# b51/ceres_mono_orb_slam2

Measured on AMD Instinct MI355X. Metric: frames/sec ORB extract+match @1241x376 + LocalBA solves/sec; 1/2/4/8 GPU, higher is better.
Workload: dtype u8; 1 GPU; KITTI 1241x376, 2000 features/frame requested (nfeatures = 2000), 8 levels, ORB extract + brute-force Hamming match vs previous frame (ratio 0.9, TH_LOW 50, rotation histogram); frames_per_launch=256, streams=2

## Files before the change

ceres_mono_orb_slam2_amd/csrc/orb_extractor.hip:

```cpp
#include <hip/hip_runtime.h>
#include <cmath>
#include <cstdint>
#include <cstdlib>
#include <atomic>
#include <vector>
#include <algorithm>
#include <new>
#include <type_traits>

#include "common.h"
#include "orb_pattern_data.h"

namespace orbhip {

static const int PATCH_SIZE = 31, HALF_PATCH = 15, EDGE_THRESHOLD = 19;
static const int MAX_LEVELS = 16;
static const int MAX_INI = 64;
static const int KEYCAP_MAX = 1 << 23;

struct LevelDev {
  int w, h;
  int pitch;
  int bpitch;
  long long pyr_off;
// ... 276 lines not shown
template <int JJ>
__device__ __forceinline__ void fast_tile_load(const uint8_t* base, uint8_t* tile, int lane, int ndw, int W4, uint32_t inv, uint32_t pitch) {
  if constexpr (JJ < FAST_TILE_LOADS) {
    if (64 * JJ >= ndw) return;
    const uint32_t k = (uint32_t)lane + 64u * JJ;
    const uint32_t row = __umul24(k, inv) >> 16;
    const uint32_t goff = __umul24(row, pitch) + 4u * (k - __umul24(row, (uint32_t)W4));
    if ((int)k < ndw)
      __builtin_amdgcn_global_load_lds((const void __attribute__((address_space(1)))*)(base + goff),
                                       (void __attribute__((address_space(3)))*)(tile + 256 * JJ), 4, 0, 0);
    fast_tile_load<JJ + 1>(base, tile, lane, ndw, W4, inv, pitch);
  }
}

#define FAST_WPB 1
#ifndef FAST_CPW
#define FAST_CPW 1
#endif
template <bool NARROW> struct FastMask;
template <> struct FastMask<true> {
  typedef uint32_t type;
  static __device__ __forceinline__ int popc(uint32_t m) { return __popc(m); }
  static __device__ __forceinline__ int ffs0(uint32_t m) { return __ffs((int)m) - 1; }
};
template <> struct FastMask<false> {
  typedef unsigned long long type;
  static __device__ __forceinline__ int popc(unsigned long long m) { return __popcll(m); }
  static __device__ __forceinline__ int ffs0(unsigned long long m) { return __ffsll((long long)m) - 1; }
};
template <bool NARROW>
__global__ __launch_bounds__(64 * FAST_WPB) void k_fast_cells(GeomDev G, const CellDesc* __restrict__ cells,
                                                   const uint8_t* __restrict__ img0, long long img_frame_bytes,
                                                   const uint8_t* __restrict__ pyr, int* __restrict__ cell_cnt,
                                                   uint32_t* __restrict__ cell_kps, int iniTh, int minTh, int lds_per_wave, int xcd_map) {
  extern __shared__ __attribute__((aligned(16))) uint8_t smem_all[];
  const int TP = G.tile_pitch;
  const int plane = (G.tile_h * TP + 15) & ~15;
  const int lane = threadIdx.x & 63;
  typedef typename FastMask<NARROW>::type mask_t;
  int f = blockIdx.y, bxi = blockIdx.x;
  if (xcd_map) {
    const uint32_t lin = blockIdx.y * gridDim.x + blockIdx.x, x = lin & 7u, i = lin >> 3;
    const uint32_t q = i / gridDim.x;
    f = (int)(x + 8u * q); bxi = (int)(i - q * gridDim.x);
  }
  const int wv = FAST_WPB == 1 ? 0 : (int)(threadIdx.x >> 6);
  uint8_t* smem = smem_all + (size_t)wv * lds_per_wave;
  for (int rep = 0; rep < FAST_CPW; rep++) {
  const int ci = (bxi * FAST_WPB + wv) * FAST_CPW + rep;
  if (ci >= G.ncells_total) return;
  uint8_t* tile = smem;
  uint8_t* score = smem + plane;
  mask_t* keep = (mask_t*)(score + plane);
  mask_t* k20 = keep + 64;
  int* qcnt = (int*)(k20 + 64);
  unsigned short* queue = (unsigned short*)(qcnt + 4);
  FAST_STAMP_INIT;
  const CellDesc c = cells[ci];
  const LevelDev& L = G.lv[c.level];
  const uint8_t* src = level_ptr(G, c.level, f, img0, img_frame_bytes, pyr);
  const int tw = c.x1 - c.x0, th = c.y1 - c.y0;
  const int iw = tw - 6, ih = th - 6;
  const uint8_t* cell_base = src + (long long)c.y0 * L.pitch + c.x0;
  const uint32_t bsh = (uint32_t)((size_t)cell_base & 3);
  const uint8_t* base_al = cell_base - bsh;
  const uint8_t* tileb = tile + bsh;
  for (int i = lane; i < plane >> 4; i += 64) ((uint4*)score)[i] = make_uint4(0u, 0u, 0u, 0u);
  keep[lane] = 0; k20[lane] = 0;
  if (lane == 0) *qcnt = 0;
  {
    const int W4 = TP >> 2, ndw = th * W4;
    const uint32_t inv = (65536u + (uint32_t)W4 - 1u) / (uint32_t)W4;
    fast_tile_load<0>(base_al, tile, lane, ndw, W4, inv, (uint32_t)L.pitch);
    __builtin_amdgcn_s_waitcnt(0);
  }
  __builtin_amdgcn_fence(__ATOMIC_ACQ_REL, "workgroup"); __builtin_amdgcn_wave_barrier();
  FAST_STAMP(0);
  int qn = 0;
  {
    const bool narrow = NARROW || iw <= 32;
    const int RW = narrow ? 8 : 4;
    const int g = narrow ? (lane & 7) : (lane & 15), lr = narrow ? (lane >> 3) : (lane >> 4);
    const int ix4 = 4 * g;
// ... 431 lines not shown
    OCT_STAMP(6);
    if (L >= N || L == prev) break;
    if (!final_phase && L + 3 * nToExpand > N) final_phase = true;
  }
  __syncthreads();
  unsigned int* best = (unsigned int*)cc;
  for (int p = tid; p < L; p += OCT_TPB) best[p] = 0;
  __syncthreads();
  for (int k0 = tid; k0 < n; k0 += OCT_TPB * OCT_U) {
    uint32_t keyv[OCT_U]; int pv[OCT_U];
#pragma unroll
    for (int u = 0; u < OCT_U; u++) { const int k = min(k0 + OCT_TPB * u, n - 1); pv[u] = (int)KN[k]; keyv[u] = K[k]; }
    asm volatile("" : "+v"(pv[0]), "+v"(pv[1]), "+v"(pv[2]), "+v"(pv[3]), "+v"(pv[4]), "+v"(pv[5]), "+v"(pv[6]), "+v"(pv[7]),
                      "+v"(keyv[0]), "+v"(keyv[1]), "+v"(keyv[2]), "+v"(keyv[3]), "+v"(keyv[4]), "+v"(keyv[5]), "+v"(keyv[6]), "+v"(keyv[7]));
#pragma unroll
    for (int u = 0; u < OCT_U; u++) if (k0 + OCT_TPB * u < n) atomicMax(&best[pv[u]], ((keyv[u] >> 24) << 24) | (0xFFFFFFu - (unsigned)(k0 + OCT_TPB * u)));
  }
  __syncthreads();
  for (int p = tid; p < L; p += OCT_TPB) {
    if (p < G.sel_cap) SEL[p] = K[0xFFFFFFu - (best[p] & 0xFFFFFFu)];
  }
  if (tid == 0) {
    sel_cnt[f * G.nlevels + level] = L;
    if (L > G.sel_cap) atomicOr(&status[f], 2);
  }
  OCT_STAMP(7);
  OCT_STAMP_END;
}
template <bool WIDE, bool GMEM>
__global__ __launch_bounds__(OCT_TPB) __attribute__((amdgpu_waves_per_eu(8, 8))) void k_octree(GeomDev G, const int* __restrict__ cell_cnt,
                                                const uint32_t* __restrict__ cell_kps, uint32_t* __restrict__ keys,
                                                unsigned short* __restrict__ knode, uint32_t* __restrict__ sel,
                                                int* __restrict__ sel_cnt, int* __restrict__ nkeys_out,
                                                int* __restrict__ status, uint8_t* __restrict__ gnodes, size_t gnodes_stride) {
  octree_body<WIDE, GMEM>(G, cell_cnt, cell_kps, keys, knode, sel, sel_cnt, nkeys_out, status, gnodes, gnodes_stride, (int)blockIdx.x, (int)blockIdx.y);
}
__global__ __launch_bounds__(OCT_TPB) void k_octree_pair(GeomDev G, const int* __restrict__ cell_cnt, const uint32_t* __restrict__ cell_kps,
                                                         uint32_t* __restrict__ keys, unsigned short* __restrict__ knode, uint32_t* __restrict__ sel,
                                                         int* __restrict__ sel_cnt, int* __restrict__ nkeys_out, int* __restrict__ status) {
  const int bx = (int)blockIdx.x, f = (int)blockIdx.y;
  if (bx < G.nlevels) octree_body<false, false>(G, cell_cnt, cell_kps, keys, knode, sel, sel_cnt, nkeys_out, status, nullptr, 0, bx, f);
  else octree_body<true, false>(G, cell_cnt, cell_kps, keys, knode, sel, sel_cnt, nkeys_out, status, nullptr, 0, bx - G.nlevels, f);
}

#define BLUR_TW 128
#define BLUR_TH 64
#if !defined(BLUR_COL_SLIDE) || !defined(ORBHIP_EXPERIMENTS)
#undef BLUR_COL_SLIDE
#define BLUR_COL_SLIDE 0
#endif
__device__ __forceinline__ int reflect101(int i, int n) {
  if (n == 1) return 0;
  while (i < 0 || i >= n) { if (i < 0) i = -i; else i = 2 * (n - 1) - i; }
  return i;
}
template <int VAR>
__global__ __launch_bounds__(256) void k_blur7(GeomDev G, const BlurTile* __restrict__ tiles,
                                               const uint8_t* __restrict__ img0, long long img_frame_bytes,
                                               const uint8_t* __restrict__ pyr, uint8_t* __restrict__ blur) {
  __shared__ __attribute__((aligned(16))) unsigned short s_mid[BLUR_TH + 6][BLUR_TW];
  const BlurTile t = tiles[blockIdx.x];
  const int f = blockIdx.y, tid = threadIdx.x;
  const LevelDev& L = G.lv[t.level];
  const uint8_t* src = level_ptr(G, t.level, f, img0, img_frame_bytes, pyr);
  uint8_t* dst = blur + (long long)f * G.blur_frame_bytes + L.blur_off;
  const int x0 = t.tx * BLUR_TW, y0 = t.ty * BLUR_TH;
  const int cg = tid & 31, rr = tid >> 5;
  const int xo = x0 + 4 * cg;
// ... 440 lines not shown
using namespace orbhip;

static std::atomic<unsigned long long> g_ctx_generation{0};
struct orbx_ctx {
  const unsigned long long generation = ++g_ctx_generation;
  int nfeatures, nlevels, iniTh, minTh, device;
  double scaleFactor;
  std::vector<float> scale, inv_scale, sigma2, inv_sigma2;
  std::vector<int> quota, umax;
  float atan_p[4], factorPI;
  int w = 0, h = 0, stride = 0, nframes = 0;
  GeomDev G;
  std::vector<CellDesc> cells;
  std::vector<BlurTile> btiles, mtiles, mtiles1;
  DevBuf d_cells, d_btiles, d_mtiles, d_mtiles1, d_tab;
  int blur_mfma = 1;
  std::vector<size_t> tab_xofs, tab_ialpha, tab_yofs, tab_ibeta;
  struct RmHost { size_t oW = 0, oC = 0, oC0 = 0, oRow = 0; int nchunks = 0, nblocks = 0; bool ok = false; };
  std::vector<RmHost> rm;
  int resize_mfma = 1;
  size_t tab_cone = 0; int cone_wgs = 0, cone_buf0 = 0, cone_bufk = 0; size_t cone_lds = 0;
  DevBuf d_pyr, d_blur, d_cellcnt, d_cellkps, d_keys, d_knode, d_sel, d_selcnt, d_nkeys, d_status, d_octnodes;
  DevBuf d_img, d_out;
  void* h_pin = nullptr; size_t h_bytes = 0;
  size_t fast_lds = 0, octree_lds = 0, octree_lds_wide = 0;
  bool octree_wide = false;
  int fast_xcd = 1;
  bool fast_narrow = false;
  int desc_xcd = 1;
  bool octree_gmem = false;
  size_t octree_row = 0;
  const uint8_t* last_img0 = nullptr; long long last_img_frame_bytes = 0; int last_nframes = 0;
  bool const_uploaded = false;
  bool profiling = false;
  std::vector<hipEvent_t> prof_events, side_events;
  hipStream_t side = nullptr;
  hipStream_t side_hi = nullptr;
  hipEvent_t ev_fork = nullptr, ev_join = nullptr;
  int lone_side_mode = 0;
  int blur_variant = 0;
  int overlap_blur = -1;
};

static int build_tables(orbx_ctx* c) {
  const int nl = c->nlevels;
  c->scale.resize(nl); c->sigma2.resize(nl); c->inv_scale.resize(nl); c->inv_sigma2.resize(nl);
  c->scale[0] = 1.0f; c->sigma2[0] = 1.0f;
  for (int i = 1; i < nl; i++) {
    c->scale[i] = (float)(c->scale[i - 1] * c->scaleFactor);
    c->sigma2[i] = c->scale[i] * c->scale[i];
  }
  for (int i = 0; i < nl; i++) { c->inv_scale[i] = 1.0f / c->scale[i]; c->inv_sigma2[i] = 1.0f / c->sigma2[i]; }
  c->quota.resize(nl);
  float factor = (float)(1.0f / c->scaleFactor);
  float nDesired = c->nfeatures * (1 - factor) / (1 - (float)std::pow((double)factor, (double)nl));
  int sum = 0;
  for (int l = 0; l < nl - 1; l++) { c->quota[l] = cv_round(nDesired); sum += c->quota[l]; nDesired *= factor; }
  c->quota[nl - 1] = std::max(c->nfeatures - sum, 0);
  c->umax.assign(HALF_PATCH + 1, 0);
  int v, v0, vmax = (int)std::floor(HALF_PATCH * std::sqrt(2.f) / 2 + 1);
  int vmin = (int)std::ceil(HALF_PATCH * std::sqrt(2.f) / 2);
  const double hp2 = HALF_PATCH * HALF_PATCH;
  for (v = 0; v <= vmax; ++v) c->umax[v] = cv_round(std::sqrt(hp2 - v * v));
  for (v = HALF_PATCH, v0 = 0; v >= vmin; --v) {
    while (c->umax[v0] == c->umax[v0 + 1]) ++v0;
    c->umax[v] = v0;
    ++v0;
  }
  const float k = (float)(180.0 / 3.14159265358979323846);
  c->atan_p[0] = 0.9997878412794807f * k; c->atan_p[1] = -0.3258083974640975f * k;
  c->atan_p[2] = 0.1555786518463281f * k; c->atan_p[3] = -0.04432655554792128f * k;
// ... 199 lines not shown
              const int ux0 = Bx[4 * (k + 1)], ux1 = std::min<int>(Bx[4 * (k + 1) + 2], G.lv[k + 1].w), uy0 = Bx[4 * (k + 1) + 1], uy1 = Bx[4 * (k + 1) + 3];
              auto cy = [&](int v) { return std::min(std::max(v, 0), Hk - 1); };
              int nx0 = xo[ux0], nx1 = std::min(xo[ux1 - 1] + 1, Wk - 1) + 1, ny0 = cy(yo[uy0]), ny1 = cy(yo[uy1 - 1] + 1) + 1;
              for (int y = uy0; y < uy1; y++) { ny0 = std::min(ny0, cy(yo[y])); ny1 = std::max(ny1, cy(yo[y] + 1) + 1); }
              for (int x = ux0; x < ux1; x++) { nx0 = std::min(nx0, xo[x]); nx1 = std::max(nx1, std::min(xo[x] + 1, Wk - 1) + 1); }
              bx0 = nx0; bx1 = nx1; by0 = ny0; by1 = ny1;
              if (k >= 1) {
                bx0 = std::min(bx0, (int)((long long)i * Wk / ntx)); bx1 = std::max(bx1, (int)((long long)(i + 1) * Wk / ntx));
                by0 = std::min(by0, (int)((long long)j * Hk / nty)); by1 = std::max(by1, (int)((long long)(j + 1) * Hk / nty));
              }
            }
            if (k >= 1) { bx0 &= ~3; bx1 = std::min(round_up(bx1, 4), round_up(Wk, 4)); }
            Bx[4 * k] = (short)bx0; Bx[4 * k + 1] = (short)by0; Bx[4 * k + 2] = (short)bx1; Bx[4 * k + 3] = (short)by1;
            const int bytes = (bx1 - bx0) * (by1 - by0);
            if (k >= 1 && (bx1 - bx0 > 256 || by1 - by0 > 256)) ok = false;
            if (k == 0 && bytes > CONE_TPB * CONE_SRC_PT) ok = false;
            if (k == 0) buf0 = std::max(buf0, bytes); else { bufk = std::max(bufk, bytes); tb += 8 * (size_t)(bx1 - bx0) + 16 * (size_t)(by1 - by0); }
          }
          tabmax = std::max(tabmax, tb);
        }
      buf0 = round_up(buf0, 16); bufk = round_up(bufk, 16);
      const size_t lds = (size_t)buf0 + 2 * (size_t)bufk + tabmax + 64;
      if (ok && lds <= 96 * 1024) {
        size_t off = (tab.size() + 15) / 16 * 16;
        tab.resize(off + boxes.size() * 2);
        std::memcpy(tab.data() + off, boxes.data(), boxes.size() * 2);
        c->tab_cone = off; c->cone_wgs = ntx * nty; c->cone_buf0 = buf0; c->cone_bufk = bufk; c->cone_lds = lds;
      }
    }
    G.pyr_frame_bytes = (pyr_off + 255) / 256 * 256;
    G.blur_frame_bytes = (blur_off + 255) / 256 * 256;
    c->fast_narrow = tile_w - 6 <= 32;
    c->fast_lds = (size_t)round_up((int)((size_t)2 * round_up(G.tile_h * G.tile_pitch, 16) + 2 * 64 * (c->fast_narrow ? 4 : 8) + 16 + (size_t)2 * std::max(tile_w - 6, 1) * std::max(tile_h - 6, 1) + 16), 16);
    c->octree_wide = false;
    for (int l = 0; l < c->nlevels; l++) c->octree_wide = c->octree_wide || G.lv[l].kcap > 65535;
    c->octree_lds = octree_lds_bytes(G.node_cap, G.max_cells_level, false, false);
    c->octree_lds_wide = octree_lds_bytes(G.node_cap, G.max_cells_level, true, false);
    c->octree_gmem = (c->octree_wide ? c->octree_lds_wide : c->octree_lds) > 160 * 1024;
    c->octree_row = (size_t)round_up((int)octree_lds_bytes(G.node_cap, G.max_cells_level, true, true), 256);
    ORBHIP_REQUIRE(G.node_cap <= 32760, ORBHIP_EINVAL, "nfeatures too large: more than 32752 keypoints in one level (16-bit node indices)");
    if (int rc = c->d_cells.ensure(std::max<size_t>(c->cells.size(), 1) * sizeof(CellDesc))) return rc;
    if (int rc = c->d_btiles.ensure(c->btiles.size() * sizeof(BlurTile))) return rc;
    if (int rc = c->d_mtiles.ensure(c->mtiles.size() * sizeof(BlurTile))) return rc;
    if (int rc = c->d_mtiles1.ensure(c->mtiles1.size() * sizeof(BlurTile))) return rc;
    if (int rc = c->d_tab.ensure(std::max<size_t>(tab.size(), 16))) return rc;
    if (!c->cells.empty()) ORBHIP_CHECK_HIP(hipMemcpy(c->d_cells.p, c->cells.data(), c->cells.size() * sizeof(CellDesc), hipMemcpyHostToDevice));
    ORBHIP_CHECK_HIP(hipMemcpy(c->d_btiles.p, c->btiles.data(), c->btiles.size() * sizeof(BlurTile), hipMemcpyHostToDevice));
    ORBHIP_CHECK_HIP(hipMemcpy(c->d_mtiles.p, c->mtiles.data(), c->mtiles.size() * sizeof(BlurTile), hipMemcpyHostToDevice));
    ORBHIP_CHECK_HIP(hipMemcpy(c->d_mtiles1.p, c->mtiles1.data(), c->mtiles1.size() * sizeof(BlurTile), hipMemcpyHostToDevice));
    if (!tab.empty()) ORBHIP_CHECK_HIP(hipMemcpy(c->d_tab.p, tab.data(), tab.size(), hipMemcpyHostToDevice));
    if (!c->octree_gmem && c->octree_lds > 64 * 1024)
      if (int rc = raise_dynamic_lds((const void*)k_octree<false, false>, c->device, c->octree_lds)) return rc;
    if (!c->octree_gmem && c->octree_wide && c->octree_lds_wide > 64 * 1024)
      if (int rc = raise_dynamic_lds((const void*)k_octree<true, false>, c->device, c->octree_lds_wide)) return rc;
    c->w = w; c->h = h; c->stride = stride; c->nframes = 0;
  }
  if (!c->const_uploaded) {
    ORBHIP_CHECK_HIP(hipMemcpyToSymbol(HIP_SYMBOL(c_pattern), ORB_BIT_PATTERN_31, 1024));
    ORBHIP_CHECK_HIP(hipMemcpyToSymbol(HIP_SYMBOL(c_umax), c->umax.data(), 16 * sizeof(int)));
    {
      std::vector<int8_t> T((size_t)2 * 7 * 64 * 16, 0);
      for (int var = 0; var < 2; var++) {
        const int taps[7] = {18, 34, var ? 48 : 49, var ? 56 : 55, var ? 48 : 49, 34, 18};
        for (int q = 0; q < 7; q++)
          for (int lane = 0; lane < 64; lane++)
            for (int j = 0; j < 16; j++) {
// ... 10 lines not shown
  const size_t B = (size_t)nframes;
  if (int rc = c->d_pyr.ensure(std::max<size_t>(B * G.pyr_frame_bytes, 256))) return rc;
  if (int rc = c->d_blur.ensure(B * G.blur_frame_bytes)) return rc;
  if (int rc = c->d_cellcnt.ensure(std::max<size_t>(B * G.ncells_total * 4, 16))) return rc;
  if (int rc = c->d_cellkps.ensure(std::max<size_t>(B * G.ncells_total * (size_t)G.cell_cap * 4, 16))) return rc;
  if (int rc = c->d_keys.ensure(B * G.keys_per_frame * 4)) return rc;
  if (int rc = c->d_knode.ensure(B * G.keys_per_frame * 2)) return rc;
  if (int rc = c->d_sel.ensure(B * nl * G.sel_cap * 4)) return rc;
  if (c->octree_gmem) { if (int rc = c->d_octnodes.ensure(B * nl * c->octree_row)) return rc; }
  if (int rc = c->d_selcnt.ensure(B * nl * 4)) return rc;
  if (int rc = c->d_nkeys.ensure(B * nl * 4)) return rc;
  if (int rc = c->d_status.ensure(B * 4)) return rc;
  c->nframes = nframes;
  return 0;
}

static int run_batch(orbx_ctx* c, const uint8_t* d_imgs, int w, int h, int stride, size_t frame_stride,
                     int nframes, orbx_keypoint* d_kps, uint8_t* d_desc, int cap, int32_t* d_counts,
                     hipStream_t st) {
  void (*blur_k)(GeomDev, const BlurTile*, const uint8_t*, long long, const uint8_t*, uint8_t*) =
      c->blur_mfma ? (c->blur_variant ? k_blur7_mfma<1> : k_blur7_mfma<0>) : (c->blur_variant ? k_blur7<1> : k_blur7<0>);

  ORBHIP_CHECK_HIP(hipSetDevice(c->device));
  if (int rc = prepare(c, w, h, stride, nframes)) return rc;
  const GeomDev& G = c->G;
  const int nl = c->nlevels;
  uint8_t* pyr = c->d_pyr.as<uint8_t>();
  const bool blur_short = c->blur_mfma && nframes < 4;
  const unsigned n_btiles = (unsigned)(c->blur_mfma ? (blur_short ? c->mtiles1.size() : c->mtiles.size()) : c->btiles.size());
  const BlurTile* d_btl = c->blur_mfma ? (blur_short ? c->d_mtiles1.as<BlurTile>() : c->d_mtiles.as<BlurTile>()) : c->d_btiles.as<BlurTile>();
  auto mark = [&]() { if (c->profiling) { hipEvent_t e; if (hipEventCreate(&e) == hipSuccess) { (void)hipEventRecord(e, st); c->prof_events.push_back(e); } } };
  static const bool cone_on = []() { const char* e = ORBHIP_EXP_ENV("ORBHIP_EXTRACT_CONE"); return !(e && e[0] == '0'); }();
  const bool cone = cone_on && nframes == 1 && c->cone_wgs > 0;
  if (!cone) ORBHIP_CHECK_HIP(hipMemsetAsync(c->d_status.p, 0, (size_t)nframes * 4, st));
  mark();
  if (cone) {
    ConeArgs ca; std::memset(&ca, 0, sizeof(ca));
    const uint8_t* T = c->d_tab.as<uint8_t>();
    ca.nl = nl; ca.spitch0 = G.lv[0].pitch; ca.buf0 = c->cone_buf0; ca.bufk = c->cone_bufk;
    for (int l = 1; l < nl; l++) {
      ConeLevel& L = ca.lv[l];
      L.sw = G.lv[l - 1].w; L.sh = G.lv[l - 1].h; L.dw = G.lv[l].w; L.dh = G.lv[l].h; L.dpitch = G.lv[l].pitch; L.doff = G.lv[l].pyr_off;
      L.xtab = (const uint2*)(T + c->tab_xofs[l]); L.yofs = (const int*)(T + c->tab_yofs[l]); L.ibeta = (const short*)(T + c->tab_ibeta[l]);
    }
    if (c->cone_lds > 64 * 1024)
      if (int rc = raise_dynamic_lds((const void*)k_pyr_cone, c->device, c->cone_lds)) return rc;
    hipLaunchKernelGGL(k_pyr_cone, dim3(c->cone_wgs), dim3(CONE_TPB), c->cone_lds, st, ca, (const short*)(T + c->tab_cone), d_imgs, pyr, c->d_status.as<int>());
  }
  for (int l = 1; l < nl && !cone; l++) {
    const LevelDev& S = G.lv[l - 1];
    const LevelDev& D = G.lv[l];
    const uint8_t* src = (l == 1) ? d_imgs : pyr + S.pyr_off;
    long long sframe = (l == 1) ? (long long)frame_stride : G.pyr_frame_bytes;
    const uint8_t* T = c->d_tab.as<uint8_t>();
    if (c->resize_mfma && (size_t)l < c->rm.size() && c->rm[l].ok && nframes <= 65535) {
      const orbx_ctx::RmHost& M = c->rm[l];
      RmLevel R; R.tab = T; R.oW = M.oW; R.oC = M.oC; R.oC0 = M.oC0; R.oRow = M.oRow; R.nchunks = M.nchunks; R.nblocks = M.nblocks; R.sw = S.w; R.sh = S.h; R.dw = D.w; R.dh = D.h;
      const int ntx = (M.nchunks + 3) / 4, ntb = (M.nblocks + RM_RB - 1) / RM_RB;
      hipLaunchKernelGGL(k_resize_mfma, dim3(ntx * ntb, nframes), dim3(256), 0, st, R, src, S.pitch, sframe, pyr + D.pyr_off, D.pitch, G.pyr_frame_bytes, ntx);
      continue;
    }
    dim3 grid((D.w + 255) / 256, (D.h + 4 * RS_ROWS - 1) / (4 * RS_ROWS), nframes), block(64, 4);
    hipLaunchKernelGGL(k_resize, grid, block, 0, st, src, S.pitch, sframe, S.w, S.h, pyr + D.pyr_off, D.pitch,
                       G.pyr_frame_bytes, D.w, D.h, (const uint2*)(T + c->tab_xofs[l]), (const int*)(T + c->tab_yofs[l]),
                       (const short*)(T + c->tab_ibeta[l]));
  }
  int side_mode = c->ev_fork ? (c->overlap_blur >= 0 ? c->overlap_blur : (nframes >= 8 ? 1 : (nframes == 1 ? c->lone_side_mode : 0))) : 0;
  static const bool side_prio_all = []() { const char* v = std::getenv("ORBHIP_SIDE_PRIORITY"); return v && v[0] == '1'; }();
  hipStream_t side_st = nullptr;
  if (side_mode) {
    const bool want_hi = (nframes == 1 && c->lone_side_mode) || side_prio_all;
    if (want_hi && !c->side_hi) {
      int lo = 0, hi = 0;
      if (!(hipDeviceGetStreamPriorityRange(&lo, &hi) == hipSuccess && hi != lo && hipStreamCreateWithPriority(&c->side_hi, hipStreamNonBlocking, hi) == hipSuccess)) c->side_hi = nullptr;
    }
    if (want_hi && c->side_hi) side_st = c->side_hi;
    else {
      if (!c->side && hipStreamCreateWithFlags(&c->side, hipStreamNonBlocking) != hipSuccess) c->side = nullptr;
      side_st = c->side;
    }
    if (!side_st) side_mode = 0;
  }
  c->lone_side_mode = 0;
  auto launch_blur_side = [&]() -> int {
    ORBHIP_CHECK_HIP(hipEventRecord(c->ev_fork, st));
    ORBHIP_CHECK_HIP(hipStreamWaitEvent(side_st, c->ev_fork, 0));
    hipEvent_t sb = nullptr, se = nullptr;
    if (c->profiling) { (void)hipEventCreate(&sb); (void)hipEventCreate(&se); (void)hipEventRecord(sb, side_st); }
    hipLaunchKernelGGL(blur_k, dim3(n_btiles, nframes), dim3(256), 0, side_st, G,
                       d_btl, d_imgs, (long long)frame_stride, pyr, c->d_blur.as<uint8_t>());
    if (c->profiling) { (void)hipEventRecord(se, side_st); c->side_events.push_back(sb); c->side_events.push_back(se); }
    ORBHIP_CHECK_HIP(hipEventRecord(c->ev_join, side_st));
    return 0;
  };
  if (side_mode == 1) { if (int rc = launch_blur_side()) return rc; }
  mark();
  if (G.ncells_total > 0) {
    if (c->fast_narrow)
      hipLaunchKernelGGL(k_fast_cells<true>, dim3((G.ncells_total + FAST_WPB * FAST_CPW - 1) / (FAST_WPB * FAST_CPW), nframes), dim3(64 * FAST_WPB), c->fast_lds * FAST_WPB, st, G,
                         c->d_cells.as<CellDesc>(), d_imgs, (long long)frame_stride, pyr, c->d_cellcnt.as<int>(),
                         c->d_cellkps.as<uint32_t>(), c->iniTh, c->minTh, (int)c->fast_lds, (c->fast_xcd && nframes % 8 == 0) ? 1 : 0);
    else
      hipLaunchKernelGGL(k_fast_cells<false>, dim3((G.ncells_total + FAST_WPB * FAST_CPW - 1) / (FAST_WPB * FAST_CPW), nframes), dim3(64 * FAST_WPB), c->fast_lds * FAST_WPB, st, G,
                         c->d_cells.as<CellDesc>(), d_imgs, (long long)frame_stride, pyr, c->d_cellcnt.as<int>(),
                         c->d_cellkps.as<uint32_t>(), c->iniTh, c->minTh, (int)c->fast_lds, (c->fast_xcd && nframes % 8 == 0) ? 1 : 0);
  }
  mark();
  if (side_mode == 2) ORBHIP_CHECK_HIP(hipEventRecord(c->ev_fork, st));
  if (!c->octree_gmem && c->octree_wide && nframes == 1) {
    const size_t lds2 = std::max(c->octree_lds, c->octree_lds_wide);
    if (lds2 > 64 * 1024)
      if (int rc = raise_dynamic_lds((const void*)k_octree_pair, c->device, lds2)) return rc;
    hipLaunchKernelGGL(k_octree_pair, dim3(2 * nl, 1), dim3(OCT_TPB), lds2, st, G, c->d_cellcnt.as<int>(), c->d_cellkps.as<uint32_t>(), c->d_keys.as<uint32_t>(),
                       c->d_knode.as<unsigned short>(), c->d_sel.as<uint32_t>(), c->d_selcnt.as<int>(), c->d_nkeys.as<int>(), c->d_status.as<int>());
  } else if (!c->octree_gmem) {
    hipLaunchKernelGGL((k_octree<false, false>), dim3(nl, nframes), dim3(OCT_TPB), c->octree_lds, st, G, c->d_cellcnt.as<int>(),
                       c->d_cellkps.as<uint32_t>(), c->d_keys.as<uint32_t>(), c->d_knode.as<unsigned short>(),
                       c->d_sel.as<uint32_t>(), c->d_selcnt.as<int>(), c->d_nkeys.as<int>(), c->d_status.as<int>(), (uint8_t*)nullptr, (size_t)0);
    if (c->octree_wide)
      hipLaunchKernelGGL((k_octree<true, false>), dim3(nl, nframes), dim3(OCT_TPB), c->octree_lds_wide, st, G, c->d_cellcnt.as<int>(),
                         c->d_cellkps.as<uint32_t>(), c->d_keys.as<uint32_t>(), c->d_knode.as<unsigned short>(),
                         c->d_sel.as<uint32_t>(), c->d_selcnt.as<int>(), c->d_nkeys.as<int>(), c->d_status.as<int>(), (uint8_t*)nullptr, (size_t)0);
  } else {
    hipLaunchKernelGGL((k_octree<false, true>), dim3(nl, nframes), dim3(OCT_TPB), 0, st, G, c->d_cellcnt.as<int>(),
                       c->d_cellkps.as<uint32_t>(), c->d_keys.as<uint32_t>(), c->d_knode.as<unsigned short>(),
                       c->d_sel.as<uint32_t>(), c->d_selcnt.as<int>(), c->d_nkeys.as<int>(), c->d_status.as<int>(), c->d_octnodes.as<uint8_t>(), c->octree_row);
    if (c->octree_wide)
      hipLaunchKernelGGL((k_octree<true, true>), dim3(nl, nframes), dim3(OCT_TPB), 0, st, G, c->d_cellcnt.as<int>(),
                         c->d_cellkps.as<uint32_t>(), c->d_keys.as<uint32_t>(), c->d_knode.as<unsigned short>(),
                         c->d_sel.as<uint32_t>(), c->d_selcnt.as<int>(), c->d_nkeys.as<int>(), c->d_status.as<int>(), c->d_octnodes.as<uint8_t>(), c->octree_row);
  }
  if (side_mode == 2) {
    ORBHIP_CHECK_HIP(hipStreamWaitEvent(side_st, c->ev_fork, 0));
    hipEvent_t sb = nullptr, se = nullptr;
    if (c->profiling) { (void)hipEventCreate(&sb); (void)hipEventCreate(&se); (void)hipEventRecord(sb, side_st); }
    hipLaunchKernelGGL(blur_k, dim3(n_btiles, nframes), dim3(256), 0, side_st, G,
                       d_btl, d_imgs, (long long)frame_stride, pyr, c->d_blur.as<uint8_t>());
    if (c->profiling) { (void)hipEventRecord(se, side_st); c->side_events.push_back(sb); c->side_events.push_back(se); }
    ORBHIP_CHECK_HIP(hipEventRecord(c->ev_join, side_st));
  }
  mark();
  if (side_mode == 0) hipLaunchKernelGGL(blur_k, dim3(n_btiles, nframes), dim3(256), 0, st, G,
                                         d_btl, d_imgs, (long long)frame_stride, pyr, c->d_blur.as<uint8_t>());
  else ORBHIP_CHECK_HIP(hipStreamWaitEvent(st, c->ev_join, 0));
  mark();
  hipLaunchKernelGGL(k_describe, dim3(G.desc_blocks, nframes), dim3(64 * DESC_WPB), 0, st, G, c->d_sel.as<uint32_t>(),
                     c->d_selcnt.as<int>(), c->d_status.as<int>(), d_imgs, (long long)frame_stride, pyr,
                     c->d_blur.as<uint8_t>(), d_kps, d_desc, cap, d_counts, c->atan_p[0], c->atan_p[1],
                     c->atan_p[2], c->atan_p[3], c->factorPI, (c->desc_xcd && nframes % 8 == 0) ? 1 : 0);
  mark();
  ORBHIP_CHECK_HIP(hipGetLastError());
  c->last_img0 = d_imgs; c->last_img_frame_bytes = (long long)frame_stride; c->last_nframes = nframes;
  return 0;
}

extern "C" {

int orbx_create(int nfeatures, float scale_factor, int nlevels, int ini_th_fast, int min_th_fast, int device,
                orbx_ctx** out) {
  ORBHIP_REQUIRE(out != nullptr, ORBHIP_EINVAL, "out is NULL");
  ORBHIP_REQUIRE(nfeatures > 0 && nlevels >= 1 && nlevels <= MAX_LEVELS && scale_factor > 1.0f, ORBHIP_EINVAL,
                 "bad extractor parameters");
  ORBHIP_REQUIRE(min_th_fast >= 1 && ini_th_fast >= min_th_fast && ini_th_fast <= 254, ORBHIP_EINVAL,
                 "FAST thresholds must satisfy 1 <= min <= ini <= 254");
  int ndev = 0;
  if (hipGetDeviceCount(&ndev) != hipSuccess || ndev <= 0) { set_error("no HIP device available (the HIP path has no CPU fallback)"); return ORBHIP_ENODEV; }
  ORBHIP_REQUIRE(device >= 0 && device < ndev, ORBHIP_EINVAL, "device ordinal out of range");
  orbx_ctx* c = new (std::nothrow) orbx_ctx();
  ORBHIP_REQUIRE(c != nullptr, ORBHIP_ENOMEM, "out of host memory");
  c->nfeatures = nfeatures; c->scaleFactor = scale_factor; c->nlevels = nlevels;
  c->iniTh = ini_th_fast; c->minTh = min_th_fast; c->device = device;
  build_tables(c);
  (void)hipSetDevice(device);
  if (hipEventCreateWithFlags(&c->ev_fork, hipEventDisableTiming) != hipSuccess) c->ev_fork = nullptr;
  if (c->ev_fork && hipEventCreateWithFlags(&c->ev_join, hipEventDisableTiming) != hipSuccess) { (void)hipEventDestroy(c->ev_fork); c->ev_fork = nullptr; c->ev_join = nullptr; }
  if (const char* e = std::getenv("ORBHIP_BLUR_MFMA")) c->blur_mfma = atoi(e) != 0;
  if (const char* e = std::getenv("ORBHIP_RESIZE_MFMA")) c->resize_mfma = atoi(e) != 0;
  if (const char* e = ORBHIP_EXP_ENV("ORBHIP_OVERLAP_BLUR")) c->overlap_blur = atoi(e);
  if (const char* e = ORBHIP_EXP_ENV("ORBHIP_DESC_XCD")) c->desc_xcd = atoi(e);
  if (const char* e = ORBHIP_EXP_ENV("ORBHIP_FAST_XCD")) c->fast_xcd = atoi(e);
  *out = c;
  return 0;
}

int orbx_destroy(orbx_ctx* c) {
  if (!c) return 0;
  DevBuf* bufs[] = {&c->d_cells, &c->d_btiles, &c->d_mtiles, &c->d_mtiles1, &c->d_tab, &c->d_pyr, &c->d_blur, &c->d_cellcnt, &c->d_cellkps,
                    &c->d_keys, &c->d_knode, &c->d_sel, &c->d_selcnt, &c->d_nkeys, &c->d_status, &c->d_img,
                    &c->d_out, &c->d_octnodes};
  for (DevBuf* b : bufs) b->release();
  if (c->h_pin) (void)hipHostFree(c->h_pin);
  if (c->side) { (void)hipStreamSynchronize(c->side); (void)hipStreamDestroy(c->side); }
  if (c->side_hi) { (void)hipStreamSynchronize(c->side_hi); (void)hipStreamDestroy(c->side_hi); }
  if (c->ev_fork) (void)hipEventDestroy(c->ev_fork);
  if (c->ev_join) (void)hipEventDestroy(c->ev_join);
  delete c;
  return 0;
}

#ifdef ORBHIP_OCT_PROF
int orbx_debug_oct_prof(unsigned long long* out , int reset) {
  ORBHIP_CHECK_HIP(hipDeviceSynchronize());
  ORBHIP_CHECK_HIP(hipMemcpyFromSymbol(out, HIP_SYMBOL(g_oct_prof), sizeof(unsigned long long) * MAX_LEVELS * 16));
  if (reset) { std::vector<unsigned long long> z((size_t)MAX_LEVELS * 16, 0ull); ORBHIP_CHECK_HIP(hipMemcpyToSymbol(HIP_SYMBOL(g_oct_prof), z.data(), z.size() * 8)); }
  return 0;
}
#endif

#ifdef ORBHIP_FAST_PROF
int orbx_debug_fast_prof(unsigned long long* out8) {
  ORBHIP_CHECK_HIP(hipDeviceSynchronize());
  std::vector<unsigned int> h((size_t)FAST_PROF_WAVES * 8);
  ORBHIP_CHECK_HIP(hipMemcpyFromSymbol(h.data(), HIP_SYMBOL(g_fast_prof), h.size() * 4));
  for (int k = 0; k < 8; k++) out8[k] = 0;
  for (size_t w = 0; w < FAST_PROF_WAVES; w++) if (h[8 * w + 7]) { for (int k = 0; k < 5; k++) out8[k] += h[8 * w + k]; out8[7]++; }
  return 0;
}
#endif

int orbx_set_profiling(orbx_ctx* c, int enable) {
  ORBHIP_REQUIRE(c != nullptr, ORBHIP_EINVAL, "ctx is NULL");
  for (hipEvent_t e : c->prof_events) (void)hipEventDestroy(e);
  for (hipEvent_t e : c->side_events) (void)hipEventDestroy(e);
  c->prof_events.clear(); c->side_events.clear();
  c->profiling = enable != 0;
  return 0;
}

int orbx_get_stage_ms(orbx_ctx* c, float* ms, int* ncalls) {
  ORBHIP_REQUIRE(c && ms && ncalls, ORBHIP_EINVAL, "NULL argument");
  ORBHIP_CHECK_HIP(hipSetDevice(c->device));
  for (int s = 0; s < 5; s++) ms[s] = 0.f;
  const size_t n = c->prof_events.size() / 6;
  if (n) ORBHIP_CHECK_HIP(hipEventSynchronize(c->prof_events.back()));
  for (size_t k = 0; k < n; k++)
    for (int s = 0; s < 5; s++) {
      float t = 0.f;
      ORBHIP_CHECK_HIP(hipEventElapsedTime(&t, c->prof_events[6 * k + s], c->prof_events[6 * k + s + 1]));
      ms[s] += t;
    }
  if (c->side_events.size() == 2 * n && n) {
    ms[3] = 0.f;
    ORBHIP_CHECK_HIP(hipEventSynchronize(c->side_events.back()));
    for (size_t k = 0; k < n; k++) { float t = 0.f; ORBHIP_CHECK_HIP(hipEventElapsedTime(&t, c->side_events[2 * k], c->side_events[2 * k + 1])); ms[3] += t; }
  }
  *ncalls = (int)n;
  for (hipEvent_t e : c->prof_events) (void)hipEventDestroy(e);
  for (hipEvent_t e : c->side_events) (void)hipEventDestroy(e);
  c->prof_events.clear(); c->side_events.clear();
  return 0;
}

int orbx_get_levels(const orbx_ctx* c) { return c ? c->nlevels : ORBHIP_EINVAL; }
int orbx_set_opencv_variant(orbx_ctx* c, int blur_variant) {
  ORBHIP_REQUIRE(c && (blur_variant == ORBX_CV_BLUR_8BIT || blur_variant == ORBX_CV_BLUR_FIXED16), ORBHIP_EINVAL, "unknown OpenCV variant");
  c->blur_variant = blur_variant;
  return 0;
}

int orbx_get_tables(const orbx_ctx* c, float* scale, float* inv_scale, float* sigma2, float* inv_sigma2,
                    int32_t* fpl) {
  ORBHIP_REQUIRE(c != nullptr, ORBHIP_EINVAL, "ctx is NULL");
  for (int i = 0; i < c->nlevels; i++) {
    if (scale) scale[i] = c->scale[i];
    if (inv_scale) inv_scale[i] = c->inv_scale[i];
    if (sigma2) sigma2[i] = c->sigma2[i];
    if (inv_sigma2) inv_sigma2[i] = c->inv_sigma2[i];
    if (fpl) fpl[i] = c->quota[i];
  }
  return 0;
}

int orbx_max_keypoints(const orbx_ctx* c) {
  if (!c) return ORBHIP_EINVAL;
  int s = 0;
  for (int q : c->quota) s += std::max(q + 3, 4 * MAX_INI);
  return s;
}

int orbx_extract_batch_device(orbx_ctx* c, const uint8_t* d_imgs, int w, int h, int stride, size_t frame_stride,
                              int nframes, orbx_keypoint* d_kps, uint8_t* d_desc, int cap, int32_t* d_counts,
                              void* stream) {
// ... 122 lines not shown
```

Baseline: 162,400 frames/s.

## Overlap level-0 FAST and octree on side stream with remaining pyramid build

Splits the pyramid levels into two groups. Once level 0 (and level 1) of the pyramid are built, FAST detection and octree selection for the first group run on the side stream while the main stream keeps building the smaller levels and then processes the rest. The goal is to overlap the serial pyramid-resize chain with feature detection on batched launches (nframes >= 8). The cost is extra launches and events, plus contention between the two streams for compute units.

```diff
diff --git a/ceres_mono_orb_slam2_amd/csrc/orb_extractor.hip b/ceres_mono_orb_slam2_amd/csrc/orb_extractor.hip
--- a/ceres_mono_orb_slam2_amd/csrc/orb_extractor.hip
+++ b/ceres_mono_orb_slam2_amd/csrc/orb_extractor.hip
@@ -332,7 +332,8 @@
 __global__ __launch_bounds__(64 * FAST_WPB) void k_fast_cells(GeomDev G, const CellDesc* __restrict__ cells,
                                                    const uint8_t* __restrict__ img0, long long img_frame_bytes,
                                                    const uint8_t* __restrict__ pyr, int* __restrict__ cell_cnt,
-                                                   uint32_t* __restrict__ cell_kps, int iniTh, int minTh, int lds_per_wave, int xcd_map) {
+                                                   uint32_t* __restrict__ cell_kps, int iniTh, int minTh, int lds_per_wave, int xcd_map,
+                                                   int cell0, int cell_end) {
   extern __shared__ __attribute__((aligned(16))) uint8_t smem_all[];
   const int TP = G.tile_pitch;
   const int plane = (G.tile_h * TP + 15) & ~15;
@@ -347,8 +348,8 @@
   const int wv = FAST_WPB == 1 ? 0 : (int)(threadIdx.x >> 6);
   uint8_t* smem = smem_all + (size_t)wv * lds_per_wave;
   for (int rep = 0; rep < FAST_CPW; rep++) {
-  const int ci = (bxi * FAST_WPB + wv) * FAST_CPW + rep;
-  if (ci >= G.ncells_total) return;
+  const int ci = cell0 + (bxi * FAST_WPB + wv) * FAST_CPW + rep;
+  if (ci >= cell_end) return;
   uint8_t* tile = smem;
   uint8_t* score = smem + plane;
   mask_t* keep = (mask_t*)(score + plane);
@@ -846,8 +847,8 @@
                                                 const uint32_t* __restrict__ cell_kps, uint32_t* __restrict__ keys,
                                                 unsigned short* __restrict__ knode, uint32_t* __restrict__ sel,
                                                 int* __restrict__ sel_cnt, int* __restrict__ nkeys_out,
-                                                int* __restrict__ status, uint8_t* __restrict__ gnodes, size_t gnodes_stride) {
-  octree_body<WIDE, GMEM>(G, cell_cnt, cell_kps, keys, knode, sel, sel_cnt, nkeys_out, status, gnodes, gnodes_stride, (int)blockIdx.x, (int)blockIdx.y);
+                                                int* __restrict__ status, uint8_t* __restrict__ gnodes, size_t gnodes_stride, int level0) {
+  octree_body<WIDE, GMEM>(G, cell_cnt, cell_kps, keys, knode, sel, sel_cnt, nkeys_out, status, gnodes, gnodes_stride, level0 + (int)blockIdx.x, (int)blockIdx.y);
 }
 __global__ __launch_bounds__(OCT_TPB) void k_octree_pair(GeomDev G, const int* __restrict__ cell_cnt, const uint32_t* __restrict__ cell_kps,
                                                          uint32_t* __restrict__ keys, unsigned short* __restrict__ knode, uint32_t* __restrict__ sel,
@@ -1354,11 +1355,18 @@
   size_t octree_row = 0;
   const uint8_t* last_img0 = nullptr; long long last_img_frame_bytes = 0; int last_nframes = 0;
   bool const_uploaded = false;
+  struct LevelGroup { int level0, nlevels, cell0, ncells, after; };
+  std::vector<LevelGroup> groups;
+  int level_split = 1;
   bool profiling = false;
-  std::vector<hipEvent_t> prof_events, side_events;
+  std::vector<hipEvent_t> prof_events;
+  struct SideSpan { int stage; hipEvent_t b, e; };
+  std::vector<SideSpan> side_spans;
+  std::vector<uint8_t> prof_side_blur;
   hipStream_t side = nullptr;
   hipStream_t side_hi = nullptr;
   hipEvent_t ev_fork = nullptr, ev_join = nullptr;
+  hipEvent_t ev_g0 = nullptr, ev_pyr = nullptr;
   int lone_side_mode = 0;
   int blur_variant = 0;
   int overlap_blur = -1;
@@ -1624,6 +1632,14 @@
     G.blur_frame_bytes = (blur_off + 255) / 256 * 256;
     c->fast_narrow = tile_w - 6 <= 32;
     c->fast_lds = (size_t)round_up((int)((size_t)2 * round_up(G.tile_h * G.tile_pitch, 16) + 2 * 64 * (c->fast_narrow ? 4 : 8) + 16 + (size_t)2 * std::max(tile_w - 6, 1) * std::max(tile_h - 6, 1) + 16), 16);
+    c->groups.clear();
+    {
+      const int nl0 = (c->level_split > 0 && c->level_split < c->nlevels) ? c->level_split : c->nlevels;
+      for (int l0 = 0; l0 < c->nlevels; l0 = (l0 == 0 ? nl0 : c->nlevels)) {
+        const int l1 = l0 == 0 ? nl0 : c->nlevels;
+        c->groups.push_back({l0, l1 - l0, G.lv[l0].cell_begin, G.lv[l1 - 1].cell_begin + G.lv[l1 - 1].ncells - G.lv[l0].cell_begin, std::max(l1 - 1, 1)});
+      }
+    }
     c->octree_wide = false;
     for (int l = 0; l < c->nlevels; l++) c->octree_wide = c->octree_wide || G.lv[l].kcap > 65535;
     c->octree_lds = octree_lds_bytes(G.node_cap, G.max_cells_level, false, false);
@@ -1700,6 +1716,57 @@
   auto mark = [&]() { if (c->profiling) { hipEvent_t e; if (hipEventCreate(&e) == hipSuccess) { (void)hipEventRecord(e, st); c->prof_events.push_back(e); } } };
   static const bool cone_on = []() { const char* e = ORBHIP_EXP_ENV("ORBHIP_EXTRACT_CONE"); return !(e && e[0] == '0'); }();
   const bool cone = cone_on && nframes == 1 && c->cone_wgs > 0;
+  int side_mode = c->ev_fork ? (c->overlap_blur >= 0 ? c->overlap_blur : (nframes >= 8 ? 1 : (nframes == 1 ? c->lone_side_mode : 0))) : 0;
+  static const bool side_prio_all = []() { const char* v = std::getenv("ORBHIP_SIDE_PRIORITY"); return v && v[0] == '1'; }();
+  hipStream_t side_st = nullptr;
+  if (side_mode) {
+    const bool want_hi = (nframes == 1 && c->lone_side_mode) || side_prio_all;
+    if (want_hi && !c->side_hi) {
+      int lo = 0, hi = 0;
+      if (!(hipDeviceGetStreamPriorityRange(&lo, &hi) == hipSuccess && hi != lo && hipStreamCreateWithPriority(&c->side_hi, hipStreamNonBlocking, hi) == hipSuccess)) c->side_hi = nullptr;
+    }
+    if (want_hi && c->side_hi) side_st = c->side_hi;
+    else {
+      if (!c->side && hipStreamCreateWithFlags(&c->side, hipStreamNonBlocking) != hipSuccess) c->side = nullptr;
+      side_st = c->side;
+    }
+    if (!side_st) side_mode = 0;
+  }
+  c->lone_side_mode = 0;
+  auto span_begin = [&](hipEvent_t& sb, hipEvent_t& se) { sb = se = nullptr; if (c->profiling) { (void)hipEventCreate(&sb); (void)hipEventCreate(&se); (void)hipEventRecord(sb, side_st); } };
+  auto span_end = [&](int stage, hipEvent_t sb, hipEvent_t se) { if (c->profiling) { (void)hipEventRecord(se, side_st); c->side_spans.push_back({stage, sb, se}); } };
+  auto launch_blur_on_side = [&]() {
+    hipEvent_t sb, se;
+    span_begin(sb, se);
+    hipLaunchKernelGGL(blur_k, dim3(n_btiles, nframes), dim3(256), 0, side_st, G,
+                       d_btl, d_imgs, (long long)frame_stride, pyr, c->d_blur.as<uint8_t>());
+    span_end(3, sb, se);
+  };
+  auto launch_fast = [&](hipStream_t s, const orbx_ctx::LevelGroup& g) {
+    if (g.ncells <= 0) return;
+    const dim3 grid((g.ncells + FAST_WPB * FAST_CPW - 1) / (FAST_WPB * FAST_CPW), nframes);
+    auto k = c->fast_narrow ? k_fast_cells<true> : k_fast_cells<false>;
+    hipLaunchKernelGGL(k, grid, dim3(64 * FAST_WPB), c->fast_lds * FAST_WPB, s, G,
+                       c->d_cells.as<CellDesc>(), d_imgs, (long long)frame_stride, pyr, c->d_cellcnt.as<int>(),
+                       c->d_cellkps.as<uint32_t>(), c->iniTh, c->minTh, (int)c->fast_lds, (c->fast_xcd && nframes % 8 == 0) ? 1 : 0,
+                       g.cell0, g.cell0 + g.ncells);
+  };
+  auto launch_octree = [&](hipStream_t s, const orbx_ctx::LevelGroup& g) {
+    const dim3 grid(g.nlevels, nframes);
+    uint8_t* gn = c->octree_gmem ? c->d_octnodes.as<uint8_t>() : (uint8_t*)nullptr;
+    const size_t gs = c->octree_gmem ? c->octree_row : (size_t)0;
+    auto go = [&](auto k, size_t lds) {
+      hipLaunchKernelGGL(k, grid, dim3(OCT_TPB), lds, s, G, c->d_cellcnt.as<int>(), c->d_cellkps.as<uint32_t>(), c->d_keys.as<uint32_t>(),
+                         c->d_knode.as<unsigned short>(), c->d_sel.as<uint32_t>(), c->d_selcnt.as<int>(), c->d_nkeys.as<int>(),
+                         c->d_status.as<int>(), gn, gs, g.level0);
+    };
+    bool wide = false;
+    for (int l = g.level0; l < g.level0 + g.nlevels; l++) wide = wide || G.lv[l].kcap > 65535;
+    if (!c->octree_gmem) { go(k_octree<false, false>, c->octree_lds); if (wide) go(k_octree<true, false>, c->octree_lds_wide); }
+    else { go(k_octree<false, true>, 0); if (wide) go(k_octree<true, true>, 0); }
+  };
+  const bool split = side_mode == 1 && nframes > 1 && c->groups.size() > 1 && c->ev_g0 && c->ev_pyr;
+  const orbx_ctx::LevelGroup all_levels{0, nl, 0, G.ncells_total, 0};
   if (!cone) ORBHIP_CHECK_HIP(hipMemsetAsync(c->d_status.p, 0, (size_t)nframes * 4, st));
   mark();
   if (cone) {
@@ -1726,53 +1793,35 @@
       RmLevel R; R.tab = T; R.oW = M.oW; R.oC = M.oC; R.oC0 = M.oC0; R.oRow = M.oRow; R.nchunks = M.nchunks; R.nblocks = M.nblocks; R.sw = S.w; R.sh = S.h; R.dw = D.w; R.dh = D.h;
       const int ntx = (M.nchunks + 3) / 4, ntb = (M.nblocks + RM_RB - 1) / RM_RB;
       hipLaunchKernelGGL(k_resize_mfma, dim3(ntx * ntb, nframes), dim3(256), 0, st, R, src, S.pitch, sframe, pyr + D.pyr_off, D.pitch, G.pyr_frame_bytes, ntx);
-      continue;
-    }
-    dim3 grid((D.w + 255) / 256, (D.h + 4 * RS_ROWS - 1) / (4 * RS_ROWS), nframes), block(64, 4);
-    hipLaunchKernelGGL(k_resize, grid, block, 0, st, src, S.pitch, sframe, S.w, S.h, pyr + D.pyr_off, D.pitch,
-                       G.pyr_frame_bytes, D.w, D.h, (const uint2*)(T + c->tab_xofs[l]), (const int*)(T + c->tab_yofs[l]),
-                       (const short*)(T + c->tab_ibeta[l]));
-  }
-  int side_mode = c->ev_fork ? (c->overlap_blur >= 0 ? c->overlap_blur : (nframes >= 8 ? 1 : (nframes == 1 ? c->lone_side_mode : 0))) : 0;
-  static const bool side_prio_all = []() { const char* v = std::getenv("ORBHIP_SIDE_PRIORITY"); return v && v[0] == '1'; }();
-  hipStream_t side_st = nullptr;
-  if (side_mode) {
-    const bool want_hi = (nframes == 1 && c->lone_side_mode) || side_prio_all;
-    if (want_hi && !c->side_hi) {
-      int lo = 0, hi = 0;
-      if (!(hipDeviceGetStreamPriorityRange(&lo, &hi) == hipSuccess && hi != lo && hipStreamCreateWithPriority(&c->side_hi, hipStreamNonBlocking, hi) == hipSuccess)) c->side_hi = nullptr;
-    }
-    if (want_hi && c->side_hi) side_st = c->side_hi;
-    else {
-      if (!c->side && hipStreamCreateWithFlags(&c->side, hipStreamNonBlocking) != hipSuccess) c->side = nullptr;
-      side_st = c->side;
-    }
-    if (!side_st) side_mode = 0;
-  }
-  c->lone_side_mode = 0;
-  auto launch_blur_side = [&]() -> int {
+    } else {
+      dim3 grid((D.w + 255) / 256, (D.h + 4 * RS_ROWS - 1) / (4 * RS_ROWS), nframes), block(64, 4);
+      hipLaunchKernelGGL(k_resize, grid, block, 0, st, src, S.pitch, sframe, S.w, S.h, pyr + D.pyr_off, D.pitch,
+                         G.pyr_frame_bytes, D.w, D.h, (const uint2*)(T + c->tab_xofs[l]), (const int*)(T + c->tab_yofs[l]),
+                         (const short*)(T + c->tab_ibeta[l]));
+    }
+    if (split && l == c->groups[0].after) {
+      ORBHIP_CHECK_HIP(hipEventRecord(c->ev_g0, st));
+      ORBHIP_CHECK_HIP(hipStreamWaitEvent(side_st, c->ev_g0, 0));
+      hipEvent_t sb, se;
+      span_begin(sb, se); launch_fast(side_st, c->groups[0]); span_end(1, sb, se);
+      span_begin(sb, se); launch_octree(side_st, c->groups[0]); span_end(2, sb, se);
+    }
+  }
+  if (split) {
+    ORBHIP_CHECK_HIP(hipEventRecord(c->ev_pyr, st));
+    ORBHIP_CHECK_HIP(hipStreamWaitEvent(side_st, c->ev_pyr, 0));
+    launch_blur_on_side();
+    ORBHIP_CHECK_HIP(hipEventRecord(c->ev_join, side_st));
+  } else if (side_mode == 1) {
     ORBHIP_CHECK_HIP(hipEventRecord(c->ev_fork, st));
     ORBHIP_CHECK_HIP(hipStreamWaitEvent(side_st, c->ev_fork, 0));
-    hipEvent_t sb = nullptr, se = nullptr;
-    if (c->profiling) { (void)hipEventCreate(&sb); (void)hipEventCreate(&se); (void)hipEventRecord(sb, side_st); }
-    hipLaunchKernelGGL(blur_k, dim3(n_btiles, nframes), dim3(256), 0, side_st, G,
-                       d_btl, d_imgs, (long long)frame_stride, pyr, c->d_blur.as<uint8_t>());
-    if (c->profiling) { (void)hipEventRecord(se, side_st); c->side_events.push_back(sb); c->side_events.push_back(se); }
+    launch_blur_on_side();
     ORBHIP_CHECK_HIP(hipEventRecord(c->ev_join, side_st));
-    return 0;
-  };
-  if (side_mode == 1) { if (int rc = launch_blur_side()) return rc; }
+  }
+  if (c->profiling) c->prof_side_blur.push_back(side_mode != 0);
   mark();
-  if (G.ncells_total > 0) {
-    if (c->fast_narrow)
-      hipLaunchKernelGGL(k_fast_cells<true>, dim3((G.ncells_total + FAST_WPB * FAST_CPW - 1) / (FAST_WPB * FAST_CPW), nframes), dim3(64 * FAST_WPB), c->fast_lds * FAST_WPB, st, G,
-                         c->d_cells.as<CellDesc>(), d_imgs, (long long)frame_stride, pyr, c->d_cellcnt.as<int>(),
-                         c->d_cellkps.as<uint32_t>(), c->iniTh, c->minTh, (int)c->fast_lds, (c->fast_xcd && nframes % 8 == 0) ? 1 : 0);
-    else
-      hipLaunchKernelGGL(k_fast_cells<false>, dim3((G.ncells_total + FAST_WPB * FAST_CPW - 1) / (FAST_WPB * FAST_CPW), nframes), dim3(64 * FAST_WPB), c->fast_lds * FAST_WPB, st, G,
-                         c->d_cells.as<CellDesc>(), d_imgs, (long long)frame_stride, pyr, c->d_cellcnt.as<int>(),
-                         c->d_cellkps.as<uint32_t>(), c->iniTh, c->minTh, (int)c->fast_lds, (c->fast_xcd && nframes % 8 == 0) ? 1 : 0);
-  }
+  if (!split) launch_fast(st, all_levels);
+  else for (size_t g = 1; g < c->groups.size(); g++) launch_fast(st, c->groups[g]);
   mark();
   if (side_mode == 2) ORBHIP_CHECK_HIP(hipEventRecord(c->ev_fork, st));
   if (!c->octree_gmem && c->octree_wide && nframes == 1) {
@@ -1781,30 +1830,14 @@
       if (int rc = raise_dynamic_lds((const void*)k_octree_pair, c->device, lds2)) return rc;
     hipLaunchKernelGGL(k_octree_pair, dim3(2 * nl, 1), dim3(OCT_TPB), lds2, st, G, c->d_cellcnt.as<int>(), c->d_cellkps.as<uint32_t>(), c->d_keys.as<uint32_t>(),
                        c->d_knode.as<unsigned short>(), c->d_sel.as<uint32_t>(), c->d_selcnt.as<int>(), c->d_nkeys.as<int>(), c->d_status.as<int>());
-  } else if (!c->octree_gmem) {
-    hipLaunchKernelGGL((k_octree<false, false>), dim3(nl, nframes), dim3(OCT_TPB), c->octree_lds, st, G, c->d_cellcnt.as<int>(),
-                       c->d_cellkps.as<uint32_t>(), c->d_keys.as<uint32_t>(), c->d_knode.as<unsigned short>(),
-                       c->d_sel.as<uint32_t>(), c->d_selcnt.as<int>(), c->d_nkeys.as<int>(), c->d_status.as<int>(), (uint8_t*)nullptr, (size_t)0);
-    if (c->octree_wide)
-      hipLaunchKernelGGL((k_octree<true, false>), dim3(nl, nframes), dim3(OCT_TPB), c->octree_lds_wide, st, G, c->d_cellcnt.as<int>(),
-                         c->d_cellkps.as<uint32_t>(), c->d_keys.as<uint32_t>(), c->d_knode.as<unsigned short>(),
-                         c->d_sel.as<uint32_t>(), c->d_selcnt.as<int>(), c->d_nkeys.as<int>(), c->d_status.as<int>(), (uint8_t*)nullptr, (size_t)0);
+  } else if (!split) {
+    launch_octree(st, all_levels);
   } else {
-    hipLaunchKernelGGL((k_octree<false, true>), dim3(nl, nframes), dim3(OCT_TPB), 0, st, G, c->d_cellcnt.as<int>(),
-                       c->d_cellkps.as<uint32_t>(), c->d_keys.as<uint32_t>(), c->d_knode.as<unsigned short>(),
-                       c->d_sel.as<uint32_t>(), c->d_selcnt.as<int>(), c->d_nkeys.as<int>(), c->d_status.as<int>(), c->d_octnodes.as<uint8_t>(), c->octree_row);
-    if (c->octree_wide)
-      hipLaunchKernelGGL((k_octree<true, true>), dim3(nl, nframes), dim3(OCT_TPB), 0, st, G, c->d_cellcnt.as<int>(),
-                         c->d_cellkps.as<uint32_t>(), c->d_keys.as<uint32_t>(), c->d_knode.as<unsigned short>(),
-                         c->d_sel.as<uint32_t>(), c->d_selcnt.as<int>(), c->d_nkeys.as<int>(), c->d_status.as<int>(), c->d_octnodes.as<uint8_t>(), c->octree_row);
+    for (size_t g = 1; g < c->groups.size(); g++) launch_octree(st, c->groups[g]);
   }
   if (side_mode == 2) {
     ORBHIP_CHECK_HIP(hipStreamWaitEvent(side_st, c->ev_fork, 0));
-    hipEvent_t sb = nullptr, se = nullptr;
-    if (c->profiling) { (void)hipEventCreate(&sb); (void)hipEventCreate(&se); (void)hipEventRecord(sb, side_st); }
-    hipLaunchKernelGGL(blur_k, dim3(n_btiles, nframes), dim3(256), 0, side_st, G,
-                       d_btl, d_imgs, (long long)frame_stride, pyr, c->d_blur.as<uint8_t>());
-    if (c->profiling) { (void)hipEventRecord(se, side_st); c->side_events.push_back(sb); c->side_events.push_back(se); }
+    launch_blur_on_side();
     ORBHIP_CHECK_HIP(hipEventRecord(c->ev_join, side_st));
   }
   mark();
@@ -1842,6 +1875,11 @@
   (void)hipSetDevice(device);
   if (hipEventCreateWithFlags(&c->ev_fork, hipEventDisableTiming) != hipSuccess) c->ev_fork = nullptr;
   if (c->ev_fork && hipEventCreateWithFlags(&c->ev_join, hipEventDisableTiming) != hipSuccess) { (void)hipEventDestroy(c->ev_fork); c->ev_fork = nullptr; c->ev_join = nullptr; }
+  if (c->ev_fork) {
+    if (hipEventCreateWithFlags(&c->ev_g0, hipEventDisableTiming) != hipSuccess) c->ev_g0 = nullptr;
+    if (hipEventCreateWithFlags(&c->ev_pyr, hipEventDisableTiming) != hipSuccess) c->ev_pyr = nullptr;
+  }
+  if (const char* e = std::getenv("ORBHIP_EXTRACT_LEVEL_SPLIT")) c->level_split = std::max(0, atoi(e));
   if (const char* e = std::getenv("ORBHIP_BLUR_MFMA")) c->blur_mfma = atoi(e) != 0;
   if (const char* e = std::getenv("ORBHIP_RESIZE_MFMA")) c->resize_mfma = atoi(e) != 0;
   if (const char* e = ORBHIP_EXP_ENV("ORBHIP_OVERLAP_BLUR")) c->overlap_blur = atoi(e);
@@ -1862,6 +1900,7 @@
   if (c->side_hi) { (void)hipStreamSynchronize(c->side_hi); (void)hipStreamDestroy(c->side_hi); }
   if (c->ev_fork) (void)hipEventDestroy(c->ev_fork);
   if (c->ev_join) (void)hipEventDestroy(c->ev_join);
+  for (hipEvent_t e : {c->ev_g0, c->ev_pyr}) if (e) (void)hipEventDestroy(e);
   delete c;
   return 0;
 }
@@ -1886,11 +1925,15 @@
 }
 #endif
 
+static void clear_prof(orbx_ctx* c) {
+  for (hipEvent_t e : c->prof_events) (void)hipEventDestroy(e);
+  for (const orbx_ctx::SideSpan& sp : c->side_spans) { (void)hipEventDestroy(sp.b); (void)hipEventDestroy(sp.e); }
+  c->prof_events.clear(); c->side_spans.clear(); c->prof_side_blur.clear();
+}
+
 int orbx_set_profiling(orbx_ctx* c, int enable) {
   ORBHIP_REQUIRE(c != nullptr, ORBHIP_EINVAL, "ctx is NULL");
-  for (hipEvent_t e : c->prof_events) (void)hipEventDestroy(e);
-  for (hipEvent_t e : c->side_events) (void)hipEventDestroy(e);
-  c->prof_events.clear(); c->side_events.clear();
+  clear_prof(c);
   c->profiling = enable != 0;
   return 0;
 }
@@ -1903,19 +1946,19 @@
   if (n) ORBHIP_CHECK_HIP(hipEventSynchronize(c->prof_events.back()));
   for (size_t k = 0; k < n; k++)
     for (int s = 0; s < 5; s++) {
+      if (s == 3 && k < c->prof_side_blur.size() && c->prof_side_blur[k]) continue;
       float t = 0.f;
       ORBHIP_CHECK_HIP(hipEventElapsedTime(&t, c->prof_events[6 * k + s], c->prof_events[6 * k + s + 1]));
       ms[s] += t;
     }
-  if (c->side_events.size() == 2 * n && n) {
-    ms[3] = 0.f;
-    ORBHIP_CHECK_HIP(hipEventSynchronize(c->side_events.back()));
-    for (size_t k = 0; k < n; k++) { float t = 0.f; ORBHIP_CHECK_HIP(hipEventElapsedTime(&t, c->side_events[2 * k], c->side_events[2 * k + 1])); ms[3] += t; }
+  if (!c->side_spans.empty()) ORBHIP_CHECK_HIP(hipEventSynchronize(c->side_spans.back().e));
+  for (const orbx_ctx::SideSpan& sp : c->side_spans) {
+    float t = 0.f;
+    ORBHIP_CHECK_HIP(hipEventElapsedTime(&t, sp.b, sp.e));
+    ms[sp.stage] += t;
   }
   *ncalls = (int)n;
-  for (hipEvent_t e : c->prof_events) (void)hipEventDestroy(e);
-  for (hipEvent_t e : c->side_events) (void)hipEventDestroy(e);
-  c->prof_events.clear(); c->side_events.clear();
+  clear_prof(c);
   return 0;
 }
 
```

New measurement: 159,200 frames/s. -2.0%, worse.
